# image-rs/deflate-rs

Measured on AMD Instinct MI355X. Metric: MB/s raw input encoded (Compression::Default) + compressed size vs ref, higher is better.
Workload: dtype u8; 1 GPU; enwik8 = enwik8-like synthetic text (tests/datagen.py text_like; --enwik8 PATH takes the real file): 100000000 bytes per GPU, Compression::Default, stream-exact (P1); bytes_per_gpu=100000000, level=Compression::Default, parallelism=shard1

## Files before the change

### __graft_entry__.py

```python
import os
import subprocess
import sys

ROOT = os.path.dirname(os.path.abspath(__file__))
PKG = os.path.join(ROOT, "deflate-rs_amd")
for p in (PKG, os.path.join(ROOT, "tests")):
    if p not in sys.path:
        sys.path.insert(0, p)


def _have_hipcc():
    return os.path.exists("/opt/rocm/bin/hipcc")


def build():
    env = dict(os.environ)
    lib = os.path.join(PKG, "libmi355deflate.so")
    if _have_hipcc():
        subprocess.check_call(["make", "-C", PKG, "-s"], env=env)
        subprocess.check_call(["make", "-C", PKG, "-s", "debug"], env=env)
    elif not os.path.exists(lib):
        raise RuntimeError("hipcc not found and no prebuilt libmi355deflate.so present")
    subprocess.check_call(["make", "-C", os.path.join(ROOT, "oracle"), "-s"], env=env)
    subprocess.check_call(["make", "-C", os.path.join(ROOT, "tests", "hostsim"), "-s"], env=env)
    subprocess.check_call(["make", "-C", os.path.join(ROOT, "tests", "inflcheck"), "-s"], env=env)
    subprocess.check_call(["make", "-C", os.path.join(ROOT, "tests", "inflwrite"), "-s"], env=env)
    subprocess.check_call(["make", "-C", os.path.join(ROOT, "tests", "infltable"), "-s"], env=env)
    subprocess.check_call(["make", "-C", os.path.join(ROOT, "tests", "inflindex"), "-s"], env=env)
    subprocess.check_call(["make", "-C", os.path.join(ROOT, "tests", "inflmembers"), "-s"], env=env)
    subprocess.check_call(["make", "-C", os.path.join(ROOT, "tests", "inflbig"), "-s"], env=env)
    subprocess.check_call(["make", "-C", os.path.join(ROOT, "tests", "inflseek"), "-s"], env=env)
    subprocess.check_call(["make", "-C", os.path.join(ROOT, "tests", "inflcut"), "-s"], env=env)
    import deflate_amd

    L = deflate_amd.load()
    for name in deflate_amd.EXPORTED:
        getattr(L, name)
    assert L.mi355_deflate_version() >= 100


def smoke():
    import zlib

    import deflate_amd
    import oracle_binding as ob

    pg = os.path.join(ROOT, "tests", "golden", "ref_inputs", "pg11.txt")
    data = open(pg, "rb").read()
    ctx = deflate_amd.Context(0)
    ctx.config(deflate_amd.Context.CFG_STAGE_CLOCKS, 1)
    out = ctx.encode(data, deflate_amd.Compression.Default)
    ref = ob.encode(data, level=ob.DEFAULT)
    assert out == ref, "HIP path differs from the oracle on pg11.txt (%d vs %d bytes)" % (len(out), len(ref))
    d = zlib.decompressobj(-15)
    assert d.decompress(out) + d.flush() == data
    z = ctx.encode(data[:70000], deflate_amd.Compression.Default, wrapper=1)
    assert zlib.decompress(z) == data[:70000]
    assert z == ob.encode(data[:70000], level=ob.DEFAULT, wrapper=1)
    info = ctx.info()
    print("smoke ok: pg11.txt %d -> %d bytes, %d blocks, match %.3f ms" %
          (len(data), len(out), info["n_blocks"], info["match_ms"]))


if __name__ == "__main__":
    build()
# ... 3 lines not shown
```

### deflate-rs_amd/csrc/deflate_batch.inc

```
namespace mi355 {

struct BatchItem {
    const uint8_t* in;
    uint32_t n, K0, nb_max;
    uint32_t q1_check;
    uint32_t out_words;
    uint32_t bit_base;
    uint32_t gz_off, gz_len;
    uint32_t *M, *Mq;
    uint16_t *adv, *S, *B;
    uint32_t *E0, *tokbuf, *cnt, *xs, *badmap, *fixlist, *base, *tend, *pb, *bstart, *q13, *dtok, *ll_freq, *d_freq, *seg_ends;
    BlockTab tab;
    BlockHeader* hdr;
    BlockPlan* plan;
    DevState* st;
    uint8_t* out;
};
enum : uint32_t { BS_SORT, BS_WALK, BS_RLE, BS_ADV, BS_EMIT, BS_COMPACT, BS_HIST, BS_HEADER, BS_PACK, BS_ADLER, BS_CRC, BS_N };
struct BatchArgs {
    const BatchItem* it;
    const uint32_t* pre;
    uint32_t n_items;
};
__device__ __forceinline__ uint32_t batch_locate(const BatchArgs& a, uint32_t stage, uint32_t& local, uint32_t& count) {
    const uint32_t* pre = a.pre + (size_t)stage * (a.n_items + 1);
    const uint32_t i = __builtin_amdgcn_readfirstlane(batch_item_of(pre, a.n_items, blockIdx.x));
    local = blockIdx.x - pre[i];
    count = pre[i + 1] - pre[i];
    return i;
}
__device__ __forceinline__ HashOverride batch_no_override() { return HashOverride{0, 0, 0, 0, 0, nullptr, 0, nullptr, 0, nullptr}; }

template <int MODE>
__global__ __launch_bounds__(1024) void kb_sort(BatchArgs bat_, uint32_t dbl) {
    uint32_t local, count;
    const BatchItem& it = bat_.it[batch_locate(bat_, BS_SORT, local, count)];
    k_sort_body<MODE>(local, it.in, it.n, batch_no_override(), it.S, it.B, 0u, dbl,
                      SortInit{reinterpret_cast<uint32_t*>(it.st), (uint32_t)(sizeof(DevScalars) / 4), it.seg_ends, it.n});
}

template <bool HAS_Q, bool SINGLE>
__global__ __launch_bounds__(M3T) __attribute__((amdgpu_waves_per_eu(4, 4))) void kb_walk(BatchArgs bat_, uint32_t checks, uint32_t checks_q,
                                                                                       uint32_t split) {
    __shared__ __attribute__((aligned(256))) uint4 s_T[M3_TABLE_U4];
    __shared__ uint32_t s_next;
    uint32_t local, count;
    const BatchItem& it = bat_.it[batch_locate(bat_, BS_WALK, local, count)];
    const uint32_t e = local / split, part = local % split;
    const SegEnds sg{it.seg_ends, 1u};
    const int aligned16 = (reinterpret_cast<uintptr_t>(it.in) & 15) == 0 ? 1 : 0;
    uint32_t* const ms = split == 1 ? walk_borrows(it.tokbuf, it.K0) : nullptr;
    uint32_t* const mqs = (HAS_Q && split == 1) ? it.dtok : nullptr;
    uint32_t* const Mq = HAS_Q ? it.Mq : nullptr;
    if (MI355_SWZ_BANKS && __builtin_amdgcn_readfirstlane((int)it.B[(size_t)e * BSTRIDE + WINDOW_SIZE + 2]))
        m3_epoch<HAS_Q, true, SINGLE>(s_T, s_next, e, part, it.in, it.n, it.S, it.B, it.M, Mq, checks, checks_q, aligned16, sg,
                                      batch_no_override(), split, ms, mqs, &it.st->sort_bad);
    else
        m3_epoch<HAS_Q, false, SINGLE>(s_T, s_next, e, part, it.in, it.n, it.S, it.B, it.M, Mq, checks, checks_q, aligned16, sg,
                                       batch_no_override(), split, ms, mqs, &it.st->sort_bad);
}

template <bool RLE>
__global__ __launch_bounds__(256) void kb_nohash(BatchArgs bat_) {
    uint32_t local, count;
    const BatchItem& it = bat_.it[batch_locate(bat_, BS_RLE, local, count)];
    if (local == 0) {
        uint32_t* const sc = reinterpret_cast<uint32_t*>(it.st);
        for (uint32_t i = threadIdx.x; i < (uint32_t)(sizeof(DevScalars) / 4); i += 256) sc[i] = 0;
        if (threadIdx.x == 0) *it.seg_ends = it.n;
    }
    if (RLE) {
        k_rle_body(local, it.in, it.n, it.M, it.adv, SegEnds{it.seg_ends, 1u});
    } else {
        const uint32_t lo = local * RT, hi = local + 1 == count ? ((it.n + 64 + 3) & ~3u) : lo + RT;
        for (uint32_t i = lo + threadIdx.x * 4; i < hi; i += 256 * 4) *reinterpret_cast<uint4*>(it.M + i) = make_uint4(0, 0, 0, 0);
    }
}

__global__ __launch_bounds__(256) void kb_adv(BatchArgs bat_, ParseCfg cfg) {
    uint32_t local, count;
    const BatchItem& it = bat_.it[batch_locate(bat_, BS_ADV, local, count)];
    k_adv_body(local, it.n, it.M, cfg.use_quarter ? it.Mq : nullptr, cfg, it.adv, SegEnds{it.seg_ends, 1u}, 0u);
}

template <bool STEPS>
__global__ __launch_bounds__(256) void kb_emit(BatchArgs bat_, ParseCfg cfg) {
    constexpr int MODE = 1;
    uint32_t local, count;
    const BatchItem& it = bat_.it[batch_locate(bat_, BS_EMIT, local, count)];
    const uint8_t* in = it.in;
    uint32_t n = it.n, K = it.K0;
    const uint32_t* M = it.M;
// ... 851 lines not shown
```

### deflate-rs_amd/csrc/deflate_host.inc

```
#include <dlfcn.h>
#include <hsa/hsa.h>
#include <hsa/hsa_ext_amd.h>
#include <stdio.h>
#include <stdlib.h>
#include <string.h>

#include <algorithm>
#include <chrono>
#include <mutex>
#include <string>
#include <vector>

#include "../../include/mi355_deflate.h"

using namespace mi355;

extern "C" size_t mi355_deflate_bound_ex(size_t n, int wrapper, size_t hdr_len, size_t n_flush);

namespace {

struct Level {
    uint32_t count;
    uint64_t usize;
    uint16_t* X;
// ... 527 lines not shown
    static const bool single_env = !(getenv("MI355_M3_SINGLE") && getenv("MI355_M3_SINGLE")[0] == '0');
    const uint32_t cus = n_cu ? n_cu : 256u;
    const uint32_t split = match3_split(n_ep, n_cu);
    return WalkPlan{split, single_env && split >= MI355_M3_SPLIT_MAX && n_ep * split * 2 <= cus};
}

void launch_walk(mi355_deflate_ctx* c, hipStream_t st, const uint8_t* d_in, uint32_t n32, const uint16_t* S, Workspace& w, const ParseCfg& cfg,
                 int aligned16, SegEnds sg, const HashOverride& ov, uint32_t e_first, uint32_t ne) {
    const WalkPlan plan = walk_plan(ne, c->n_cu);
    const uint32_t split = plan.split, cq = cfg_cq(cfg);
    const bool has_q = cfg_has_q(cfg);
    uint32_t* const borrowed = walk_borrows(w.tokbuf, w.K0);
    uint32_t* const ms = split == 1 ? borrowed : nullptr;
    uint32_t* const mqs = split == 1 ? w.dtok : nullptr;
    if (MI355_SWZ_BANKS && ne * split <= M3_BOTH_UNITS) {
        const bool single = plan.single;
        const uint32_t sp = single ? split * 2 : split;
        uint32_t* const ms1 = sp == 1 ? borrowed : nullptr;
        uint32_t* const mqs1 = sp == 1 ? w.dtok : nullptr;
#define MI355_BOTH(Q, SNG, mq, mqs, cqv)                                                                                       \
    hipLaunchKernelGGL((k_match3_both<Q, SNG>), dim3(ne * sp), dim3(M3T), 0, st, d_in, n32, S, w.buckets, w.M, mq, cfg.checks, cqv, \
                       aligned16, sg, ov, e_first, sp, ms1, mqs, sort_bad_flag(c))
        if (has_q && single)
            MI355_BOTH(true, true, w.Mq, mqs1, cq);
        else if (has_q)
            MI355_BOTH(true, false, w.Mq, mqs1, cq);
        else if (single)
            MI355_BOTH(false, true, (uint32_t*)nullptr, (uint32_t*)nullptr, 0u);
        else
            MI355_BOTH(false, false, (uint32_t*)nullptr, (uint32_t*)nullptr, 0u);
#undef MI355_BOTH
        return;
    }
    if (has_q)
        hipLaunchKernelGGL(k_match3<true>, dim3(ne * split), dim3(M3T), 0, st, d_in, n32, S, w.buckets, w.M, w.Mq, cfg.checks, cq,
                           aligned16, sg, ov, e_first, split, ms, mqs, sort_bad_flag(c));
    else
        hipLaunchKernelGGL(k_match3<false>, dim3(ne * split), dim3(M3T), 0, st, d_in, n32, S, w.buckets, w.M, (uint32_t*)nullptr,
                           cfg.checks, 0u, aligned16, sg, ov, e_first, split, ms, (uint32_t*)nullptr, sort_bad_flag(c));
    if (MI355_SWZ_BANKS) {
        const uint32_t units = ne * split, cus = c->n_cu ? c->n_cu : 256u;
        const uint32_t grid = (MI355_SWZ_PERSISTENT && units > cus) ? cus : units;
        if (has_q)
            hipLaunchKernelGGL(k_match3_swz<true>, dim3(grid), dim3(M3T), 0, st, d_in, n32, S, w.buckets, w.M, w.Mq, cfg.checks, cq,
                               aligned16, sg, ov, e_first, units, split, ms, mqs, sort_bad_flag(c));
        else
            hipLaunchKernelGGL(k_match3_swz<false>, dim3(grid), dim3(M3T), 0, st, d_in, n32, S, w.buckets, w.M, (uint32_t*)nullptr,
                               cfg.checks, 0u, aligned16, sg, ov, e_first, units, split, ms, (uint32_t*)nullptr, sort_bad_flag(c));
    }
}

struct SegRange {
    uint32_t seg_hi;
    Piece piece;
    const uint8_t* d_in;
    uint32_t n, pos0, n_total;
    uint32_t runup0;
    SegEnds sg;
    const uint16_t* steps;
    uint32_t* E0;
    uint32_t* xs;
    uint32_t* fixlist;
    uint32_t* n_fix;
    uint32_t* scan_part;
    uint32_t* tend;
    uint32_t* pb;
};

void launch_spec_emit(hipStream_t st, const Workspace& w, const ParseCfg& cfg, const SegRange& r) {
    const SpecFix fx{r.fixlist, w.badmap, r.n_fix};
    MI355_LAUNCH_EMIT(1, r.steps, dim3(cdiv(r.seg_hi - r.piece.seg_lo, 4)), st, r.d_in, r.n, r.seg_hi, w.M, cfg.use_quarter ? w.Mq : nullptr, cfg,
                       r.steps, r.E0, w.tokbuf, w.cnt, r.pos0, r.n_total, r.sg, r.xs, fx, r.runup0, r.piece.seg_lo);
// ... 1606 lines not shown
```

### deflate-rs_amd/csrc/deflate_kernels.hip

```cpp
#include <hip/hip_runtime.h>
#include <stdint.h>

#include <type_traits>

#ifdef MI355_MATCH_STATS
__device__ unsigned long long g_mstats[16];
__device__ unsigned long long g_sstats[16];
#define MI355_STAT_DECL uint32_t stat_[8] = {0, 0, 0, 0, 0, 0, 0, 0};
#define MI355_STAT(i, v) stat_[i] += (v);
#define MI355_STAT_FLUSH(policy)                                                          \
    for (int i_ = 0; i_ < 8; i_++) atomicAdd(&g_mstats[i_], (unsigned long long)stat_[i_]); \
    atomicMax((policy).wgmax, stat_[0]);                                                  \
    if ((threadIdx.x & 63) == 0) {                                                        \
        unsigned long long t_ = wall_clock64();                                           \
        atomicMax((policy).wgend, t_);                                                    \
        atomicAdd((policy).wgsum, t_ - (policy).t0);                                      \
    }
#endif
#include "stages.h"

namespace mi355 {

struct GBytes {
    const uint8_t* d;
// ... 807 lines not shown
                very += nb <= MI355_SWZ_BANKS / 2 ? 1u : 0u;
            }
            bool banks_few = few >= 2 || very >= 1;
#ifdef MI355_DEBUG_HOOKS
            if (force_swz) banks_few = force_swz == 1u;
#endif
            Bg[(size_t)e * BSTRIDE + WINDOW_SIZE + 2] = (J >= 1024 && banks_few && dbl) ? 1 : 0;
        }
    }
    uint4* out = reinterpret_cast<uint4*>(Sg + (size_t)e * WINDOW_SIZE);
    const uint4* fin = reinterpret_cast<const uint4*>(sH);
    for (uint32_t k = tid; k < (J + 7) / 8; k += 1024) {
        const uint4 v = fin[k];
        out[k] = make_uint4(v.x << dbl, v.y << dbl, v.z << dbl, v.w << dbl);
    }
}
template <int MODE>
__global__ __launch_bounds__(1024) void k_sort(const uint8_t* __restrict__ in, uint32_t n, HashOverride ov,
                                               uint16_t* __restrict__ Sg, uint16_t* __restrict__ Bg, uint32_t e0, uint32_t dbl,
                                               SortInit init) {
    k_sort_body<MODE>(blockIdx.x, in, n, ov, Sg, Bg, e0, dbl, init);
}

#ifdef MI355_MATCH_STATS
#define M2_CNT(i, v) \
    if (((MI355_MATCH_STATS) & 2) || (i) == 0 || (i) == 4) m2c[i] += (uint32_t)(v);
#define M2_T0 uint32_t m2t = ((MI355_MATCH_STATS) & 1) ? (uint32_t)__builtin_readcyclecounter() : 0u;
#define M2_T(i)                                                      \
    if ((MI355_MATCH_STATS) & 1) {                                   \
        const uint32_t t_ = (uint32_t)__builtin_readcyclecounter();  \
        m2c[i] += t_ - m2t;                                          \
        m2t = t_;                                                    \
    }
#else
#define M2_CNT(i, v)
#define M2_T0
#define M2_T(i)
#endif

constexpr uint32_t M3T = 1024;
constexpr uint32_t M3_PAIRS = 2 * WINDOW_SIZE + 258 + 14;

template <bool SWZ>
struct PairWinT {
    const uint16_t* sb;
    uint32_t tbase;
    typedef __attribute__((address_space(3))) const uint16_t* lds_u16;
    enum : uint32_t { SH = 1 };
    __device__ uint32_t key_at(uint32_t a) const { return *(lds_u16)(SWZ ? m3_swz(a) : a); }
    __device__ void load16(uint32_t pos, uint32_t* q) const {
        typedef uint32_t u32x2 __attribute__((ext_vector_type(2)));
        u32x2 d0, d1, d2, d3, d4;
        const uint32_t a8 = (tbase + 2 * pos) & ~7u;
        if (SWZ) {
            asm volatile(
                "ds_read_b64 %0, %5\n\t"
                "ds_read_b64 %1, %6\n\t"
                "ds_read_b64 %2, %7\n\t"
                "ds_read_b64 %3, %8\n\t"
                "ds_read_b64 %4, %9\n\t"
                "s_waitcnt lgkmcnt(0)"
                : "=&v"(d0), "=&v"(d1), "=&v"(d2), "=&v"(d3), "=&v"(d4)
                : "v"(m3_swz(a8)), "v"(m3_swz(a8 + 8)), "v"(m3_swz(a8 + 16)), "v"(m3_swz(a8 + 24)), "v"(m3_swz(a8 + 32))
                : "memory");
        } else
        asm volatile(
            "ds_read_b64 %0, %5\n\t"
            "ds_read_b64 %1, %5 offset:8\n\t"
            "ds_read_b64 %2, %5 offset:16\n\t"
            "ds_read_b64 %3, %5 offset:24\n\t"
// ... 151 lines not shown
        "s_mov_b64 %[cx], exec\n\t" \
        "s_mov_b64 exec, %[cy]\n\t" \
        MF_TEST8("y", "7", "6", "5", "4", "3", "2", "1", "0") \
        "s_mov_b64 %[cy], exec\n\t" \
        "s_branch .Lmf_end%=\n\t" \
        ".Lmf_xonly%=:\n\t" \
        MF_ONE(RD8, "x", "wx", "cx", "v[56:59]", "v[60:63]", "v56", "v57", "v58", "v59", "v60", "v61", "v62", "v63") \
        "s_branch .Lmf_end%=\n\t" \
        ".Lmf_yonly%=:\n\t" \
        MF_ONE(RD8, "y", "wy", "cy", "v[64:67]", "v[68:71]", "v64", "v65", "v66", "v67", "v68", "v69", "v70", "v71") \
        ".Lmf_end%=:\n\t" \
        "s_waitcnt vmcnt(0)\n\t" \
        "s_mov_b64 exec, %[save]\n\t" \
        : MF_OPS(x, x), MF_OPS(y, y), [save] "=&s"(save), [cx] "=&s"(cx), [cy] "=&s"(cy) \
        : MF_INS(x, x), MF_INS(y, y), [sb] "s"(sb8), [wx] "s"(walkx), [wy] "s"(walky) \
        : "vcc", "scc", "memory", "v56", "v57", "v58", "v59", "v60", "v61", "v62", "v63", "v64", "v65", "v66", "v67", "v68", "v69", \
          "v70", "v71"); \
    *stillx = cx; \
    *stilly = cy; \
}
MS_STEPS_DUAL_DEF(ms_steps_dual, MF_RD8_0)
MS_STEPS_DUAL_DEF(ms_steps_dual_swz, MF_RD8_1)
#undef MF_ONE

constexpr uint32_t ADV_TILE = 1024, ADV_HALO = 260;
struct TileM {
    const uint32_t* t;
    __device__ uint32_t operator()(uint32_t r) const { return t[r]; }
};
__device__ __forceinline__ uint32_t rel_end(const SegEnds& sg, uint64_t base, uint32_t r) {
    const uint64_t e = (uint64_t)seg_end(sg, base + r) - base;
    return e > 0xFFFFFFFFull ? 0xFFFFFFFFu : (uint32_t)e;
}
template <bool HAS_Q, bool SWZ, bool SINGLE = false>
__device__ __forceinline__ void m3_epoch(uint4* s_T, uint32_t& s_next, const uint32_t e, const uint32_t part, const uint8_t* __restrict__ in, uint32_t n,
                                         const uint16_t* __restrict__ Sg, const uint16_t* __restrict__ Bg, uint32_t* __restrict__ M,
                                         uint32_t* __restrict__ Mq, uint32_t checks, uint32_t checks_q, int in_aligned16, SegEnds sg,
                                         HashOverride ov, uint32_t split, uint32_t* __restrict__ Ms, uint32_t* __restrict__ Mqs,
                                         uint32_t* __restrict__ sort_bad) {
    constexpr uint32_t pair = SINGLE ? 1u : 2u;
    const uint32_t tid = threadIdx.x, lane = tid & 63;
#ifdef MI355_MATCH_STATS
    uint32_t m2c[16] = {0, 0, 0, 0, 0, 0, 0, 0, 0, 0, 0, 0, 0, 0, 0, 0};
#endif
    M2_T0
    const uint64_t E = (uint64_t)e * WINDOW_SIZE;
    const uint64_t wbase = e ? E - WINDOW_SIZE : 0;
    const uint32_t wbytes = (uint32_t)(E - wbase) + WINDOW_SIZE + 258 + 14;
    const uint32_t tb0 = (uint32_t)(uintptr_t)(__attribute__((address_space(3))) uint4*)s_T;
    for (uint32_t w = tid; w < wbytes / 16; w += M3T) {
        const uint64_t g = wbase + 16ull * w;
        uint32_t t[5] = {0, 0, 0, 0, 0};
        if (in_aligned16 && g + 20 <= n) {
            const uint4 v = *reinterpret_cast<const uint4*>(in + g);
            t[0] = v.x;
            t[1] = v.y;
            t[2] = v.z;
            t[3] = v.w;
            t[4] = *reinterpret_cast<const uint32_t*>(in + g + 16);
        } else {
            for (int b = 0; b < 17; b++)
                if (g + b < n) t[b >> 2] |= (uint32_t)in[g + b] << (8 * (b & 3));
        }
        uint32_t o[8];
#pragma unroll
        for (int k = 0; k < 4; k++) {
            o[2 * k] = __builtin_amdgcn_perm(t[k], t[k], 0x02010100u);
            o[2 * k + 1] = __builtin_amdgcn_perm(t[k + 1], t[k], 0x04030302u);
        }
        if (SWZ) {
            typedef __attribute__((address_space(3))) uint64_t* lds_u64;
            const uint32_t a = tb0 + 32u * w;
#pragma unroll
            for (int k = 0; k < 4; k++) *(lds_u64)m3_swz(a + 8u * k) = (uint64_t)o[2 * k] | ((uint64_t)o[2 * k + 1] << 32);
        } else {
            s_T[2 * w] = make_uint4(o[0], o[1], o[2], o[3]);
            s_T[2 * w + 1] = make_uint4(o[4], o[5], o[6], o[7]);
        }
    }
    const uint32_t J = epoch_active(n, E);
    const uint32_t nbat = (J + 63) / 64;
    const uint32_t b_lo = (uint32_t)((uint64_t)nbat * part / split), b_hi = (uint32_t)((uint64_t)nbat * (part + 1) / split);
    if (tid == 0) s_next = b_lo;
    if (part == 0 && tid < 2) {
        const uint64_t p = E + J + tid;
        if (p < n && p < E + WINDOW_SIZE) {
            M[p] = 0;
            if (HAS_Q) Mq[p] = 0;
        }
    }
    __syncthreads();
    const uint32_t tbase = tb0;
    const uint32_t bias = (uint32_t)(E - wbase);
    const uint16_t* sbase = Sg + (size_t)e * WINDOW_SIZE - WINDOW_SIZE;
    const uint16_t* own = Sg + (size_t)e * WINDOW_SIZE;
    const uint16_t* Bown = Bg + (size_t)e * BSTRIDE;
    const uint16_t* Bprev = Bown - BSTRIDE;
    TileLimit lim{sg, wbase, sg.m == 1 ? (uint32_t)(sg.ends[0] - wbase) : 0u};
    M2_T(10)
    uint32_t unordered = 0;
    auto set_up = [&](const auto& win, SwG<HAS_Q>& st, uint32_t b, bool have, uint32_t* srel_out, uint32_t before0, uint32_t* last_out,
                      uint32_t skip, uint32_t budget, uint32_t budget_q) -> bool {
        const uint32_t j = b * 64 + lane;
        const bool valid = have && j < J;
        uint32_t raw = 0, srel = 0, ob = 0, pb0 = 0, pb1 = 0, prel = bias, nrel = bias;
        if (valid) {
            raw = (uint32_t)own[j];
            srel = raw >> 1;
            prel = bias + srel;
            const uint32_t v = win.load32(prel);
            const uint32_t ab = rewarm_ab(ov, E + srel, v & 0xff, (v >> 8) & 0xff);
            const uint32_t h = hash3(ab & 0xff, ab >> 8, (v >> 16) & 0xff);
            ob = Bown[h];
            if (e) {
                pb0 = Bprev[h];
// ... 29 lines not shown
            M2_CNT(2, 1)
            M2_CNT(3, __popcll(dropped))
            swg_service<decltype(run1)::value>(st, win, tbase, checks_q, dropped, any & dropped, asel, st.offb + back);
        }
    };
    uint32_t* const Mo = Ms ? Ms : M;
    uint32_t* const Mqo = Ms ? Mqs : Mq;
    const uint16_t* sb8u;
    {
        const uint64_t v = (uint64_t)(uintptr_t)(sbase - 4);
        const uint32_t lo = (uint32_t)__builtin_amdgcn_readfirstlane((int)(uint32_t)v);
        const uint32_t hi = (uint32_t)__builtin_amdgcn_readfirstlane((int)(uint32_t)(v >> 32));
        sb8u = (const uint16_t*)(uintptr_t)(((uint64_t)hi << 32) | lo);
    }
    auto walk_all = [&](auto run1) {
        constexpr bool RUN1 = decltype(run1)::value;
        const PairWinT<SWZ> win{sbase, tbase};
        uint32_t pxat = ~0u, pxm = 0, pxq = 0, pyat = ~0u, pym = 0, pyq = 0;
        for (;;) {
            uint32_t b = 0;
            if (lane == 0) b = atomicAdd(&s_next, pair);
            b = (uint32_t)__builtin_amdgcn_readfirstlane((int)b);
            if (b >= b_hi) break;
            SwG<HAS_Q> sx, sy;
            uint32_t srx, sry;
            uint32_t lastx, lasty;
            const uint32_t front = b ? (uint32_t)own[(uint32_t)__builtin_amdgcn_readfirstlane((int)(b * 64 - 1))] : 0u;
            const uint32_t half = (pair == 1u && checks >= 16u) ? checks / 2u : 0u;
            const bool vx = set_up(win, sx, b, true, &srx, front, &lastx, 0u, half ? half : checks, checks_q);
            const bool vy = half ? set_up(win, sy, b, true, &sry, front, &lasty, half, checks - half, 0u)
                                 : set_up(win, sy, b + 1, pair == 2u && b + 1 < b_hi, &sry, lastx, &lasty, 0u, checks, checks_q);
            (void)lasty;
            M2_CNT(0, 2)
            M2_T(8)
            if (pxat != ~0u) {
                Mo[E + pxat] = pxm;
                if (HAS_Q) Mqo[E + pxat] = pxq;
            }
            if (pyat != ~0u) {
                Mo[E + pyat] = pym;
                if (HAS_Q) Mqo[E + pyat] = pyq;
            }
            {
                const uint64_t dx = swg_first(sx, win, 8u), dy = swg_first(sy, win, 8u);
                if (dx) swg_service<RUN1>(sx, win, tbase, checks_q, dx, dx, sx.a0, sx.offb + 16u);
                if (dy) swg_service<RUN1>(sy, win, tbase, checks_q, dy, dy, sy.a0, sy.offb + 16u);
                M2_CNT(2, 2)
                M2_CNT(3, __popcll(dx) + __popcll(dy))
                M2_T(9)
            }
            for (;;) {
                const uint64_t wx = sx.walk, wy = sy.walk;
                if ((wx | wy) == 0) break;
                M2_CNT(1, 1)
                M2_CNT(7, __popcll(wx) + __popcll(wy))
                uint64_t cx, cy;
                if (SWZ)
                    ms_steps_dual_swz(sx, sy, sb8u, wx, wy, &cx, &cy);
                else
                    ms_steps_dual(sx, sy, sb8u, wx, wy, &cx, &cy);
                M2_T(12)
                sx.walk = cx;
                sy.walk = cy;
                uint64_t dx, dy;
                asm("s_andn2_b64 %0, %2, %3\n\ts_andn2_b64 %1, %4, %5" : "=&s"(dx), "=&s"(dy) : "s"(wx), "s"(cx), "s"(wy), "s"(cy) : "scc");
                if (dx) settle(run1, win, sx, dx);
                if (dy) settle(run1, win, sy, dy);
                M2_T(9)
            }
            swg_result(sx, &pxm, &pxq);
            swg_result(sy, &pym, &pyq);
            pxat = vx ? (Ms ? b * 64 + lane : srx) : ~0u;
            pyat = vy ? (Ms ? b * 64 + 64 + lane : sry) : ~0u;
            if (half) {
                pxm = m_len(pym) > m_len(pxm) ? pym : pxm;
                pyat = ~0u;
            }
            M2_T(13)
        }
        if (pxat != ~0u) {
            Mo[E + pxat] = pxm;
            if (HAS_Q) Mqo[E + pxat] = pxq;
        }
        if (pyat != ~0u) {
            Mo[E + pyat] = pym;
            if (HAS_Q) Mqo[E + pyat] = pyq;
        }
    };
    if (!SWZ && __builtin_amdgcn_readfirstlane((int)Bown[WINDOW_SIZE + 1]))
        walk_all(std::true_type{});
    else
        walk_all(std::false_type{});
    if (__builtin_amdgcn_ballot_w64(unordered != 0) != 0 && lane == 0) atomicOr(sort_bad, 1u);
    M2_T(11)
    if (Ms) {
        uint32_t* const lm = reinterpret_cast<uint32_t*>(s_T);
        const uint32_t cnt = (uint32_t)((uint64_t)n - E < (uint64_t)WINDOW_SIZE ? (uint64_t)n - E : (uint64_t)WINDOW_SIZE);
        for (int pass = 0; pass < (HAS_Q ? 2 : 1); pass++) {
            const uint32_t* src = pass ? Mqs : Ms;
            uint32_t* dst = pass ? Mq : M;
            __syncthreads();
            for (uint32_t j = tid; j < J; j += M3T) lm[(uint32_t)own[j] >> 1] = src[E + j];
            if (tid < 2 && J + tid < cnt) lm[J + tid] = 0;
            __syncthreads();
            for (uint32_t i = tid * 4; i < cnt; i += M3T * 4) {
                if (i + 4 <= cnt) {
                    *reinterpret_cast<uint4*>(dst + E + i) = *reinterpret_cast<const uint4*>(lm + i);
                } else {
                    for (uint32_t k = i; k < cnt; k++) dst[E + k] = lm[k];
                }
            }
        }
    }
    M2_T(14)
    M2_CNT(4, 1)
#ifdef MI355_MATCH_STATS
    if (lane == 0)
        for (int i = 0; i < 16; i++) atomicAdd(&g_mstats[i], (unsigned long long)m2c[i]);
#endif
}

constexpr uint32_t M3_TABLE_U4 = (M3_PAIRS * 2 + 255) / 256 * 16;
template <bool HAS_Q>
__global__ __launch_bounds__(M3T) __attribute__((amdgpu_waves_per_eu(4, 4))) void k_match3(const uint8_t* __restrict__ in, uint32_t n, const uint16_t* __restrict__ Sg,
                                                const uint16_t* __restrict__ Bg, uint32_t* __restrict__ M,
                                                uint32_t* __restrict__ Mq, uint32_t checks, uint32_t checks_q, int in_aligned16,
                                                SegEnds sg, HashOverride ov, uint32_t e0, uint32_t split, uint32_t* __restrict__ Ms,
                                                uint32_t* __restrict__ Mqs, uint32_t* __restrict__ sort_bad) {
    __shared__ __attribute__((aligned(256))) uint4 s_T[M3_TABLE_U4];
    __shared__ uint32_t s_next;
    const uint32_t e = e0 + blockIdx.x / split, part = blockIdx.x % split;
    if (MI355_SWZ_BANKS && __builtin_amdgcn_readfirstlane((int)Bg[(size_t)e * BSTRIDE + WINDOW_SIZE + 2])) return;
    m3_epoch<HAS_Q, false>(s_T, s_next, e, part, in, n, Sg, Bg, M, Mq, checks, checks_q, in_aligned16, sg, ov, split, Ms, Mqs, sort_bad);
}
template <bool HAS_Q>
__global__ __launch_bounds__(M3T) __attribute__((amdgpu_waves_per_eu(4, 4))) void k_match3_swz(const uint8_t* __restrict__ in, uint32_t n, const uint16_t* __restrict__ Sg,
                                                const uint16_t* __restrict__ Bg, uint32_t* __restrict__ M,
                                                uint32_t* __restrict__ Mq, uint32_t checks, uint32_t checks_q, int in_aligned16,
                                                SegEnds sg, HashOverride ov, uint32_t e0, uint32_t units, uint32_t split,
                                                uint32_t* __restrict__ Ms, uint32_t* __restrict__ Mqs, uint32_t* __restrict__ sort_bad) {
    __shared__ __attribute__((aligned(256))) uint4 s_T[M3_TABLE_U4];
    __shared__ uint32_t s_next;
#if MI355_SWZ_PERSISTENT
    for (uint32_t u = blockIdx.x; u < units; u += gridDim.x) {
        const uint32_t e = e0 + u / split;
        if (!__builtin_amdgcn_readfirstlane((int)Bg[(size_t)e * BSTRIDE + WINDOW_SIZE + 2])) continue;
        __syncthreads();
        m3_epoch<HAS_Q, true>(s_T, s_next, e, u % split, in, n, Sg, Bg, M, Mq, checks, checks_q, in_aligned16, sg, ov, split, Ms, Mqs, sort_bad);
    }
#else
    (void)units;
    const uint32_t e = e0 + blockIdx.x / split;
    if (!__builtin_amdgcn_readfirstlane((int)Bg[(size_t)e * BSTRIDE + WINDOW_SIZE + 2])) return;
    m3_epoch<HAS_Q, true>(s_T, s_next, e, blockIdx.x % split, in, n, Sg, Bg, M, Mq, checks, checks_q, in_aligned16, sg, ov, split, Ms, Mqs, sort_bad);
#endif
}

#ifndef MI355_M3_BOTH_UNITS
#define MI355_M3_BOTH_UNITS 256
#endif
constexpr uint32_t M3_BOTH_UNITS = MI355_M3_BOTH_UNITS;
template <bool HAS_Q, bool SINGLE>
__global__ __launch_bounds__(M3T) __attribute__((amdgpu_waves_per_eu(4, 4))) void k_match3_both(const uint8_t* __restrict__ in, uint32_t n, const uint16_t* __restrict__ Sg,
                                                const uint16_t* __restrict__ Bg, uint32_t* __restrict__ M,
                                                uint32_t* __restrict__ Mq, uint32_t checks, uint32_t checks_q, int in_aligned16,
                                                SegEnds sg, HashOverride ov, uint32_t e0, uint32_t split, uint32_t* __restrict__ Ms,
                                                uint32_t* __restrict__ Mqs, uint32_t* __restrict__ sort_bad) {
    __shared__ __attribute__((aligned(256))) uint4 s_T[M3_TABLE_U4];
    __shared__ uint32_t s_next;
    const uint32_t e = e0 + blockIdx.x / split, part = blockIdx.x % split;
    if (MI355_SWZ_BANKS && __builtin_amdgcn_readfirstlane((int)Bg[(size_t)e * BSTRIDE + WINDOW_SIZE + 2]))
        m3_epoch<HAS_Q, true, SINGLE>(s_T, s_next, e, part, in, n, Sg, Bg, M, Mq, checks, checks_q, in_aligned16, sg, ov, split, Ms, Mqs, sort_bad);
    else
        m3_epoch<HAS_Q, false, SINGLE>(s_T, s_next, e, part, in, n, Sg, Bg, M, Mq, checks, checks_q, in_aligned16, sg, ov, split, Ms, Mqs, sort_bad);
}

constexpr uint32_t RT = 4096;
constexpr uint32_t RLE_UNITS = RT / 16 + 17;
constexpr uint32_t RLE_BYTES = 16 + RLE_UNITS * 16;
__device__ __forceinline__ void k_rle_body(uint32_t bx_, const uint8_t* __restrict__ in, uint32_t n, uint32_t* __restrict__ R,
                                           uint16_t* __restrict__ adv, SegEnds sg) {
    __shared__ __attribute__((aligned(16))) uint8_t s[RLE_BYTES];
    __shared__ uint32_t eb[RLE_UNITS + 1];
    __shared__ __attribute__((aligned(16))) uint32_t so[RT];
    __shared__ __attribute__((aligned(16))) uint16_t sa[RT];
    const uint32_t tid = threadIdx.x;
    const uint64_t E = (uint64_t)bx_ * RT;
    const bool al = (reinterpret_cast<uintptr_t>(in) & 15) == 0;
    for (uint32_t k = tid; k < RLE_BYTES / 16; k += 256) {
        const int64_t g0 = (int64_t)E - 16 + 16 * (int64_t)k;
        uint4 v = make_uint4(0, 0, 0, 0);
        if (al && g0 >= 0 && (uint64_t)g0 + 16 <= n) {
            v = *reinterpret_cast<const uint4*>(in + g0);
        } else {
            uint32_t t[4] = {0, 0, 0, 0};
            for (int b = 0; b < 16; b++) {
                const int64_t g = g0 + b;
                if (g >= 0 && (uint64_t)g < n) t[b >> 2] |= (uint32_t)in[g] << (8 * (b & 3));
            }
            v = make_uint4(t[0], t[1], t[2], t[3]);
        }
        *reinterpret_cast<uint4*>(s + 16 * k) = v;
    }
    __syncthreads();
    auto unit_bits = [&](uint32_t u) -> uint32_t {
        const uint32_t* w = reinterpret_cast<const uint32_t*>(s + 16 * u + 12);
        const uint32_t d0 = w[0], d1 = w[1], d2 = w[2], d3 = w[3], d4 = w[4];
// ... 1669 lines not shown
```

### deflate-rs_amd/csrc/stages.h

```cpp
#ifndef MI355_DEFLATE_STAGES_H
#define MI355_DEFLATE_STAGES_H

#include <stdint.h>

#if defined(__HIPCC__)
#define MI355_HD __host__ __device__ __forceinline__
#else
#define MI355_HD inline
#endif

namespace mi355 {

enum : uint32_t {
    WINDOW_SIZE = 32768,
    MIN_MATCH = 3,
    MAX_MATCH = 258,
    TOO_FAR = 8192,
    MAX_BUFFER_LENGTH = 31744,
    MAX_STORED_BLOCK_LENGTH = 32767,
    NUM_LL = 286,
    NUM_DIST = 30,
    END_OF_BLOCK = 256,
    MAX_JUMP = 520,
    ZONE = 576,
// ... 586 lines not shown
        s.hq = s.hq | cap;
    }
    const lane_flag imp = hit & lf_of(len > s.bm1 + 1);
    const uint32_t delta = lf_me(imp) ? len - 1 - s.bm1 : 0u;
    s.bestd = lf_me(imp) ? s.prel - cpos : s.bestd;
    s.bm1 += delta;
    s.bb2 += delta << W::SH;
    s.lowa2 += delta << W::SH;
    const lane_flag full = imp & lf_of(len == s.maxlen);
    const uint32_t pr = w.key_at(tbase + ((s.prel + s.bm1) << W::SH));
    s.probe = lf_me(imp) ? pr : s.probe;
    s.offb = lf_me(hit) ? ho - 2 : s.offb;
    const lane_flag more = lf_of((int32_t)s.offb >= (int32_t)s.endb);
    const lane_flag resume = lf_and_not(hit & more, full);
    const lane_flag sw = lf_and_not(lf_and_not(dropped, resume), full) & s.has2;
    if (lf_any(sw)) {
        if (HAS_Q) s.hoq = lf_me(sw) ? s.hoq2 : s.hoq;
        s.offb = lf_me(sw) ? s.offb2 : s.offb;
        s.endb = lf_me(sw) ? s.endb2 : s.endb;
        s.bb2 = lf_me(sw) ? tbase + (s.bm1 << W::SH) : s.bb2;
        s.has2 = lf_and_not(s.has2, sw);
    }
    s.walk = s.walk | resume | sw;
}

template <bool HAS_Q>
MI355_HD void swg_result(const SwG<HAS_Q>& s, uint32_t* m, uint32_t* mq) {
    const uint32_t r = m_pack(s.bestd ? s.bm1 + 1 : 0, s.bestd);
    *m = r;
    *mq = (HAS_Q && lf_me(s.hq)) ? s.mq : r;
}

MI355_HD uint32_t m3_swz(uint32_t a) { return a ^ ((a >> 5) & 0xF8u); }

template <class Bytes>
MI355_HD uint32_t rle_run(const Bytes& by, uint64_t p, uint64_t n) {
    if (p == 0) return 0;
    uint32_t prev = by(p - 1);
    uint64_t cap = n - p < (uint64_t)MAX_MATCH ? n - p : (uint64_t)MAX_MATCH;
    uint32_t c = 0;
    while (c < cap && by(p + c) == prev) c++;
    return c;
}

struct SegEnds {
    const uint32_t* ends;
    uint32_t m;
};
MI355_HD uint32_t seg_end(const SegEnds& sg, uint64_t p) {
    if (sg.m == 1) return sg.ends[0];
    uint32_t lo = 0, hi = sg.m - 1;
    while (lo < hi) {
        uint32_t mid = (lo + hi) >> 1;
        if (sg.ends[mid] > p)
            hi = mid;
        else
            lo = mid + 1;
    }
    return sg.ends[lo];
}

struct ParseCfg {
    uint32_t mode;
    uint32_t checks;
    uint32_t lazy_lt;
    uint32_t use_quarter;
// ... 571 lines not shown
```

Baseline: 23540 MB/s.

## Prefetch match-window staging loads early and warm caches for the next epoch

The match3 kernels now issue the first window-staging load (and the run/mark flags as one combined load) before branching, stage later rounds ahead in registers, and touch the sort keys for the first batch early. After the walk, each block also issues loads that warm L2 for the epoch a stride ahead (input bytes, sort keys, bucket flags). The aim is to hide global-memory latency at the start of each epoch. The cost is extra register pressure and redundant loads, including for blocks that exit early.

```diff
diff --git a/__graft_entry__.py b/__graft_entry__.py
--- a/__graft_entry__.py
+++ b/__graft_entry__.py
@@ -31,6 +31,7 @@
     subprocess.check_call(["make", "-C", os.path.join(ROOT, "tests", "inflbig"), "-s"], env=env)
     subprocess.check_call(["make", "-C", os.path.join(ROOT, "tests", "inflseek"), "-s"], env=env)
     subprocess.check_call(["make", "-C", os.path.join(ROOT, "tests", "inflcut"), "-s"], env=env)
+    subprocess.check_call(["make", "-C", os.path.join(ROOT, "tests", "matchwarm"), "-s"], env=env)
     import deflate_amd
 
     L = deflate_amd.load()
diff --git a/deflate-rs_amd/csrc/deflate_batch.inc b/deflate-rs_amd/csrc/deflate_batch.inc
--- a/deflate-rs_amd/csrc/deflate_batch.inc
+++ b/deflate-rs_amd/csrc/deflate_batch.inc
@@ -52,12 +52,15 @@
     uint32_t* const ms = split == 1 ? walk_borrows(it.tokbuf, it.K0) : nullptr;
     uint32_t* const mqs = (HAS_Q && split == 1) ? it.dtok : nullptr;
     uint32_t* const Mq = HAS_Q ? it.Mq : nullptr;
-    if (MI355_SWZ_BANKS && __builtin_amdgcn_readfirstlane((int)it.B[(size_t)e * BSTRIDE + WINDOW_SIZE + 2]))
+    const M3Flags fl = m3_flags(it.B, e);
+    const M3Head hd = m3_head(it.in, it.n, aligned16, it.B, e, threadIdx.x);
+    const uint32_t run = fl.run;
+    if (MI355_SWZ_BANKS && __builtin_amdgcn_readfirstlane((int)fl.mark))
         m3_epoch<HAS_Q, true, SINGLE>(s_T, s_next, e, part, it.in, it.n, it.S, it.B, it.M, Mq, checks, checks_q, aligned16, sg,
-                                      batch_no_override(), split, ms, mqs, &it.st->sort_bad);
+                                      batch_no_override(), split, ms, mqs, &it.st->sort_bad, hd, run);
     else
         m3_epoch<HAS_Q, false, SINGLE>(s_T, s_next, e, part, it.in, it.n, it.S, it.B, it.M, Mq, checks, checks_q, aligned16, sg,
-                                       batch_no_override(), split, ms, mqs, &it.st->sort_bad);
+                                       batch_no_override(), split, ms, mqs, &it.st->sort_bad, hd, run);
 }
 
 template <bool RLE>
diff --git a/deflate-rs_amd/csrc/deflate_host.inc b/deflate-rs_amd/csrc/deflate_host.inc
--- a/deflate-rs_amd/csrc/deflate_host.inc
+++ b/deflate-rs_amd/csrc/deflate_host.inc
@@ -583,12 +583,13 @@
 #undef MI355_BOTH
         return;
     }
+    const uint32_t warm_stride = c->n_cu ? c->n_cu : 256u, e_end = e_first + ne;
     if (has_q)
         hipLaunchKernelGGL(k_match3<true>, dim3(ne * split), dim3(M3T), 0, st, d_in, n32, S, w.buckets, w.M, w.Mq, cfg.checks, cq,
-                           aligned16, sg, ov, e_first, split, ms, mqs, sort_bad_flag(c));
+                           aligned16, sg, ov, e_first, split, ms, mqs, sort_bad_flag(c), warm_stride, e_end);
     else
         hipLaunchKernelGGL(k_match3<false>, dim3(ne * split), dim3(M3T), 0, st, d_in, n32, S, w.buckets, w.M, (uint32_t*)nullptr,
-                           cfg.checks, 0u, aligned16, sg, ov, e_first, split, ms, (uint32_t*)nullptr, sort_bad_flag(c));
+                           cfg.checks, 0u, aligned16, sg, ov, e_first, split, ms, (uint32_t*)nullptr, sort_bad_flag(c), warm_stride, e_end);
     if (MI355_SWZ_BANKS) {
         const uint32_t units = ne * split, cus = c->n_cu ? c->n_cu : 256u;
         const uint32_t grid = (MI355_SWZ_PERSISTENT && units > cus) ? cus : units;
diff --git a/deflate-rs_amd/csrc/deflate_kernels.hip b/deflate-rs_amd/csrc/deflate_kernels.hip
--- a/deflate-rs_amd/csrc/deflate_kernels.hip
+++ b/deflate-rs_amd/csrc/deflate_kernels.hip
@@ -863,10 +863,17 @@
         m2c[i] += t_ - m2t;                                          \
         m2t = t_;                                                    \
     }
+#define M2_T_SETUP     \
+    if (pxat == ~0u && pyat == ~0u) { \
+        M2_T(15)       \
+    } else {           \
+        M2_T(8)        \
+    }
 #else
 #define M2_CNT(i, v)
 #define M2_T0
 #define M2_T(i)
+#define M2_T_SETUP
 #endif
 
 constexpr uint32_t M3T = 1024;
@@ -1084,12 +1091,126 @@
     const uint64_t e = (uint64_t)seg_end(sg, base + r) - base;
     return e > 0xFFFFFFFFull ? 0xFFFFFFFFu : (uint32_t)e;
 }
+#ifndef MI355_M3_EARLY_FLAGS
+#define MI355_M3_EARLY_FLAGS 1
+#endif
+#ifndef MI355_M3_STAGE_AHEAD
+#define MI355_M3_STAGE_AHEAD 1
+#endif
+#ifndef MI355_M3_WARM_FIRST
+#define MI355_M3_WARM_FIRST 1
+#endif
+#ifndef MI355_M3_WARM_NEXT
+#define MI355_M3_WARM_NEXT 2
+#endif
+struct M3Flags {
+    uint32_t run, mark;
+};
+__device__ __forceinline__ M3Flags m3_flags(const uint16_t* __restrict__ Bg, uint32_t e) {
+    uint32_t both;
+    __builtin_memcpy(&both, Bg + (size_t)e * BSTRIDE + WINDOW_SIZE + 1, 4);
+    return M3Flags{both & 0xffffu, both >> 16};
+}
+__device__ __forceinline__ uint64_t m3_wbase(uint32_t e) { return e ? (uint64_t)e * WINDOW_SIZE - WINDOW_SIZE : 0; }
+__device__ __forceinline__ bool m3_whole_item(uint32_t n, int in_aligned16, uint64_t g) { return in_aligned16 && g + 20 <= n; }
+__device__ __forceinline__ void m3_fetch(const uint8_t* __restrict__ in, uint32_t n, int in_aligned16, uint64_t g, uint32_t (&t)[5]) {
+    t[0] = t[1] = t[2] = t[3] = t[4] = 0;
+    if (m3_whole_item(n, in_aligned16, g)) {
+        const uint4 v = *reinterpret_cast<const uint4*>(in + g);
+        t[0] = v.x;
+        t[1] = v.y;
+        t[2] = v.z;
+        t[3] = v.w;
+        t[4] = *reinterpret_cast<const uint32_t*>(in + g + 16);
+    } else {
+        for (int b = 0; b < 17; b++)
+            if (g + b < n) t[b >> 2] |= (uint32_t)in[g + b] << (8 * (b & 3));
+    }
+}
+struct M3Head {
+    uint4 v;
+    uint32_t t4;
+    bool whole;
+};
+__device__ __forceinline__ M3Head m3_head(const uint8_t* __restrict__ in, uint32_t n, int in_aligned16, const uint16_t* __restrict__ Bg,
+                                          uint32_t e, uint32_t w, bool inside = true) {
+    M3Head h;
+    const uint64_t g = m3_wbase(e) + 16ull * w;
+    h.whole = inside && m3_whole_item(n, in_aligned16, g);
+    const uint8_t* src = h.whole ? in + g : reinterpret_cast<const uint8_t*>(Bg + (size_t)e * BSTRIDE + WINDOW_SIZE);
+    h.v = *reinterpret_cast<const uint4*>(src);
+    h.t4 = *reinterpret_cast<const uint32_t*>(src + 16);
+    return h;
+}
+constexpr uint32_t M3_ROUNDS = (M3_PAIRS / 16 + M3T - 1) / M3T;
+template <bool SWZ, uint32_t PAIR>
+__device__ __forceinline__ void m3_stage(uint32_t tb0, const uint8_t* __restrict__ in, uint32_t n, int in_aligned16,
+                                         const uint16_t* __restrict__ Sg, const uint16_t* __restrict__ Bg, uint32_t e, const M3Head& hd,
+                                         uint32_t J, uint32_t b_lo) {
+    const uint32_t tid = threadIdx.x, lane = tid & 63;
+    const uint64_t wbase = m3_wbase(e);
+    const uint32_t wbytes = (uint32_t)((uint64_t)e * WINDOW_SIZE - wbase) + WINDOW_SIZE + 258 + 14;
+    M3Head it[M3_ROUNDS];
+    it[0] = hd;
+#if MI355_M3_STAGE_AHEAD
+#pragma unroll
+    for (uint32_t r = 1; r < M3_ROUNDS; r++) it[r] = m3_head(in, n, in_aligned16, Bg, e, tid + r * M3T, tid + r * M3T < wbytes / 16);
+#endif
+#if MI355_M3_WARM_FIRST
+    const uint16_t* const se = Sg + (size_t)e * WINDOW_SIZE;
+    const uint32_t j0 = (b_lo + PAIR * (tid >> 6)) * 64 + lane;
+    const uint32_t warm_a = se[j0 < J ? j0 : 0u], warm_b = se[(PAIR == 2 && j0 + 64 < J) ? j0 + 64 : 0u];
+    const uint32_t warm_c = se[(j0 && j0 < J) ? j0 - 1 : 0u];
+#endif
+    auto put = [&](uint32_t w, const uint32_t (&t)[5]) {
+        uint32_t o[8];
+#pragma unroll
+        for (int k = 0; k < 4; k++) {
+            o[2 * k] = __builtin_amdgcn_perm(t[k], t[k], 0x02010100u);
+            o[2 * k + 1] = __builtin_amdgcn_perm(t[k + 1], t[k], 0x04030302u);
+        }
+        if (SWZ) {
+            typedef __attribute__((address_space(3))) uint64_t* lds_u64;
+            const uint32_t a = tb0 + 32u * w;
+#pragma unroll
+            for (int k = 0; k < 4; k++) *(lds_u64)m3_swz(a + 8u * k) = (uint64_t)o[2 * k] | ((uint64_t)o[2 * k + 1] << 32);
+        } else {
+            typedef uint32_t u32x4 __attribute__((ext_vector_type(4)));
+            typedef __attribute__((address_space(3))) u32x4* lds_u4;
+            *(lds_u4)(tb0 + 32u * w) = u32x4{o[0], o[1], o[2], o[3]};
+            *(lds_u4)(tb0 + 32u * w + 16u) = u32x4{o[4], o[5], o[6], o[7]};
+        }
+    };
+#pragma unroll
+    for (uint32_t r = 0; r < M3_ROUNDS; r++) {
+#if !MI355_M3_STAGE_AHEAD
+        if (r) it[r].whole = false;
+#endif
+        if (it[r].whole) {
+            const uint32_t t[5] = {it[r].v.x, it[r].v.y, it[r].v.z, it[r].v.w, it[r].t4};
+            put(tid + r * M3T, t);
+        }
+    }
+#pragma unroll
+    for (uint32_t r = 0; r < M3_ROUNDS; r++) {
+        const uint32_t w = tid + r * M3T;
+        if (w < wbytes / 16 && !it[r].whole) {
+            uint32_t t[5];
+            m3_fetch(in, n, in_aligned16, wbase + 16ull * w, t);
+            put(w, t);
+        }
+    }
+#if MI355_M3_WARM_FIRST
+    asm volatile("" ::"v"(warm_a), "v"(warm_b), "v"(warm_c));
+#endif
+}
 template <bool HAS_Q, bool SWZ, bool SINGLE = false>
 __device__ __forceinline__ void m3_epoch(uint4* s_T, uint32_t& s_next, const uint32_t e, const uint32_t part, const uint8_t* __restrict__ in, uint32_t n,
                                          const uint16_t* __restrict__ Sg, const uint16_t* __restrict__ Bg, uint32_t* __restrict__ M,
                                          uint32_t* __restrict__ Mq, uint32_t checks, uint32_t checks_q, int in_aligned16, SegEnds sg,
                                          HashOverride ov, uint32_t split, uint32_t* __restrict__ Ms, uint32_t* __restrict__ Mqs,
-                                         uint32_t* __restrict__ sort_bad) {
+                                         uint32_t* __restrict__ sort_bad, const M3Head& hd, uint32_t run_flag,
+                                         uint32_t warm_stride = 0, uint32_t e_end = 0) {
     constexpr uint32_t pair = SINGLE ? 1u : 2u;
     const uint32_t tid = threadIdx.x, lane = tid & 63;
 #ifdef MI355_MATCH_STATS
@@ -1097,42 +1218,13 @@
 #endif
     M2_T0
     const uint64_t E = (uint64_t)e * WINDOW_SIZE;
-    const uint64_t wbase = e ? E - WINDOW_SIZE : 0;
+    const uint64_t wbase = m3_wbase(e);
     const uint32_t wbytes = (uint32_t)(E - wbase) + WINDOW_SIZE + 258 + 14;
     const uint32_t tb0 = (uint32_t)(uintptr_t)(__attribute__((address_space(3))) uint4*)s_T;
-    for (uint32_t w = tid; w < wbytes / 16; w += M3T) {
-        const uint64_t g = wbase + 16ull * w;
-        uint32_t t[5] = {0, 0, 0, 0, 0};
-        if (in_aligned16 && g + 20 <= n) {
-            const uint4 v = *reinterpret_cast<const uint4*>(in + g);
-            t[0] = v.x;
-            t[1] = v.y;
-            t[2] = v.z;
-            t[3] = v.w;
-            t[4] = *reinterpret_cast<const uint32_t*>(in + g + 16);
-        } else {
-            for (int b = 0; b < 17; b++)
-                if (g + b < n) t[b >> 2] |= (uint32_t)in[g + b] << (8 * (b & 3));
-        }
-        uint32_t o[8];
-#pragma unroll
-        for (int k = 0; k < 4; k++) {
-            o[2 * k] = __builtin_amdgcn_perm(t[k], t[k], 0x02010100u);
-            o[2 * k + 1] = __builtin_amdgcn_perm(t[k + 1], t[k], 0x04030302u);
-        }
-        if (SWZ) {
-            typedef __attribute__((address_space(3))) uint64_t* lds_u64;
-            const uint32_t a = tb0 + 32u * w;
-#pragma unroll
-            for (int k = 0; k < 4; k++) *(lds_u64)m3_swz(a + 8u * k) = (uint64_t)o[2 * k] | ((uint64_t)o[2 * k + 1] << 32);
-        } else {
-            s_T[2 * w] = make_uint4(o[0], o[1], o[2], o[3]);
-            s_T[2 * w + 1] = make_uint4(o[4], o[5], o[6], o[7]);
-        }
-    }
     const uint32_t J = epoch_active(n, E);
     const uint32_t nbat = (J + 63) / 64;
     const uint32_t b_lo = (uint32_t)((uint64_t)nbat * part / split), b_hi = (uint32_t)((uint64_t)nbat * (part + 1) / split);
+    m3_stage<SWZ, pair>(tb0, in, n, in_aligned16, Sg, Bg, e, hd, J, b_lo);
     if (tid == 0) s_next = b_lo;
     if (part == 0 && tid < 2) {
         const uint64_t p = E + J + tid;
@@ -1228,7 +1320,7 @@
                                  : set_up(win, sy, b + 1, pair == 2u && b + 1 < b_hi, &sry, lastx, &lasty, 0u, checks, checks_q);
             (void)lasty;
             M2_CNT(0, 2)
-            M2_T(8)
+            M2_T_SETUP
             if (pxat != ~0u) {
                 Mo[E + pxat] = pxm;
                 if (HAS_Q) Mqo[E + pxat] = pxq;
@@ -1283,11 +1375,29 @@
             if (HAS_Q) Mqo[E + pyat] = pyq;
         }
     };
-    if (!SWZ && __builtin_amdgcn_readfirstlane((int)Bown[WINDOW_SIZE + 1]))
+    if (!SWZ && __builtin_amdgcn_readfirstlane((int)run_flag))
         walk_all(std::true_type{});
     else
         walk_all(std::false_type{});
     if (__builtin_amdgcn_ballot_w64(unordered != 0) != 0 && lane == 0) atomicOr(sort_bad, 1u);
+#if MI355_M3_WARM_NEXT
+    uint32_t warm_next = 0;
+    if (warm_stride) {
+        const M3Warm wr = m3_warm_ranges(e, e_end, n, warm_stride, split, BSTRIDE, MI355_M3_WARM_NEXT == 2);
+        if (wr.on) {
+            constexpr uint32_t LINE = 128, s_lines = M3_WARM_S * 2 / LINE;
+            const uint32_t in_lines = (uint32_t)((wr.in_hi - wr.in_lo + LINE - 1) / LINE);
+            if (tid < in_lines) {
+                warm_next = in[wr.in_lo + (uint64_t)LINE * tid];
+            } else if (tid < in_lines + 2 * s_lines) {
+                const uint32_t k = tid - in_lines;
+                warm_next = (Sg + (k < s_lines ? wr.s_lo[0] : wr.s_lo[1]))[(k % s_lines) * (LINE / 2)];
+            } else if (tid == in_lines + 2 * s_lines) {
+                warm_next = Bg[wr.b_lo];
+            }
+        }
+    }
+#endif
     M2_T(11)
     if (Ms) {
         uint32_t* const lm = reinterpret_cast<uint32_t*>(s_T);
@@ -1308,6 +1418,9 @@
             }
         }
     }
+#if MI355_M3_WARM_NEXT
+    asm volatile("" ::"v"(warm_next));
+#endif
     M2_T(14)
     M2_CNT(4, 1)
 #ifdef MI355_MATCH_STATS
@@ -1322,12 +1435,20 @@
                                                 const uint16_t* __restrict__ Bg, uint32_t* __restrict__ M,
                                                 uint32_t* __restrict__ Mq, uint32_t checks, uint32_t checks_q, int in_aligned16,
                                                 SegEnds sg, HashOverride ov, uint32_t e0, uint32_t split, uint32_t* __restrict__ Ms,
-                                                uint32_t* __restrict__ Mqs, uint32_t* __restrict__ sort_bad) {
+                                                uint32_t* __restrict__ Mqs, uint32_t* __restrict__ sort_bad, uint32_t warm_stride,
+                                                uint32_t e_end) {
     __shared__ __attribute__((aligned(256))) uint4 s_T[M3_TABLE_U4];
     __shared__ uint32_t s_next;
     const uint32_t e = e0 + blockIdx.x / split, part = blockIdx.x % split;
-    if (MI355_SWZ_BANKS && __builtin_amdgcn_readfirstlane((int)Bg[(size_t)e * BSTRIDE + WINDOW_SIZE + 2])) return;
-    m3_epoch<HAS_Q, false>(s_T, s_next, e, part, in, n, Sg, Bg, M, Mq, checks, checks_q, in_aligned16, sg, ov, split, Ms, Mqs, sort_bad);
+    const M3Flags fl = m3_flags(Bg, e);
+    if (!MI355_M3_EARLY_FLAGS && MI355_SWZ_BANKS && __builtin_amdgcn_readfirstlane((int)fl.mark)) return;
+    const M3Head hd = m3_head(in, n, in_aligned16, Bg, e, threadIdx.x);
+    if (MI355_M3_EARLY_FLAGS && MI355_SWZ_BANKS && __builtin_amdgcn_readfirstlane((int)fl.mark)) {
+        asm volatile("" ::"v"(hd.v.x), "v"(hd.t4));
+        return;
+    }
+    m3_epoch<HAS_Q, false>(s_T, s_next, e, part, in, n, Sg, Bg, M, Mq, checks, checks_q, in_aligned16, sg, ov, split, Ms, Mqs, sort_bad, hd,
+                           fl.run, warm_stride, e_end);
 }
 template <bool HAS_Q>
 __global__ __launch_bounds__(M3T) __attribute__((amdgpu_waves_per_eu(4, 4))) void k_match3_swz(const uint8_t* __restrict__ in, uint32_t n, const uint16_t* __restrict__ Sg,
@@ -1340,15 +1461,17 @@
 #if MI355_SWZ_PERSISTENT
     for (uint32_t u = blockIdx.x; u < units; u += gridDim.x) {
         const uint32_t e = e0 + u / split;
-        if (!__builtin_amdgcn_readfirstlane((int)Bg[(size_t)e * BSTRIDE + WINDOW_SIZE + 2])) continue;
+        if (!__builtin_amdgcn_readfirstlane((int)m3_flags(Bg, e).mark)) continue;
+        const M3Head hd = m3_head(in, n, in_aligned16, Bg, e, threadIdx.x);
         __syncthreads();
-        m3_epoch<HAS_Q, true>(s_T, s_next, e, u % split, in, n, Sg, Bg, M, Mq, checks, checks_q, in_aligned16, sg, ov, split, Ms, Mqs, sort_bad);
+        m3_epoch<HAS_Q, true>(s_T, s_next, e, u % split, in, n, Sg, Bg, M, Mq, checks, checks_q, in_aligned16, sg, ov, split, Ms, Mqs, sort_bad, hd, 0u);
     }
 #else
     (void)units;
     const uint32_t e = e0 + blockIdx.x / split;
-    if (!__builtin_amdgcn_readfirstlane((int)Bg[(size_t)e * BSTRIDE + WINDOW_SIZE + 2])) return;
-    m3_epoch<HAS_Q, true>(s_T, s_next, e, blockIdx.x % split, in, n, Sg, Bg, M, Mq, checks, checks_q, in_aligned16, sg, ov, split, Ms, Mqs, sort_bad);
+    if (!__builtin_amdgcn_readfirstlane((int)m3_flags(Bg, e).mark)) return;
+    const M3Head hd = m3_head(in, n, in_aligned16, Bg, e, threadIdx.x);
+    m3_epoch<HAS_Q, true>(s_T, s_next, e, blockIdx.x % split, in, n, Sg, Bg, M, Mq, checks, checks_q, in_aligned16, sg, ov, split, Ms, Mqs, sort_bad, hd, 0u);
 #endif
 }
 
@@ -1365,10 +1488,13 @@
     __shared__ __attribute__((aligned(256))) uint4 s_T[M3_TABLE_U4];
     __shared__ uint32_t s_next;
     const uint32_t e = e0 + blockIdx.x / split, part = blockIdx.x % split;
-    if (MI355_SWZ_BANKS && __builtin_amdgcn_readfirstlane((int)Bg[(size_t)e * BSTRIDE + WINDOW_SIZE + 2]))
-        m3_epoch<HAS_Q, true, SINGLE>(s_T, s_next, e, part, in, n, Sg, Bg, M, Mq, checks, checks_q, in_aligned16, sg, ov, split, Ms, Mqs, sort_bad);
+    const M3Flags fl = m3_flags(Bg, e);
+    const M3Head hd = m3_head(in, n, in_aligned16, Bg, e, threadIdx.x);
+    const uint32_t run = fl.run;
+    if (MI355_SWZ_BANKS && __builtin_amdgcn_readfirstlane((int)fl.mark))
+        m3_epoch<HAS_Q, true, SINGLE>(s_T, s_next, e, part, in, n, Sg, Bg, M, Mq, checks, checks_q, in_aligned16, sg, ov, split, Ms, Mqs, sort_bad, hd, run);
     else
-        m3_epoch<HAS_Q, false, SINGLE>(s_T, s_next, e, part, in, n, Sg, Bg, M, Mq, checks, checks_q, in_aligned16, sg, ov, split, Ms, Mqs, sort_bad);
+        m3_epoch<HAS_Q, false, SINGLE>(s_T, s_next, e, part, in, n, Sg, Bg, M, Mq, checks, checks_q, in_aligned16, sg, ov, split, Ms, Mqs, sort_bad, hd, run);
 }
 
 constexpr uint32_t RT = 4096;
diff --git a/deflate-rs_amd/csrc/stages.h b/deflate-rs_amd/csrc/stages.h
--- a/deflate-rs_amd/csrc/stages.h
+++ b/deflate-rs_amd/csrc/stages.h
@@ -642,6 +642,31 @@
 }
 
 MI355_HD uint32_t m3_swz(uint32_t a) { return a ^ ((a >> 5) & 0xF8u); }
+
+constexpr uint32_t M3_WARM_S = 2048;
+constexpr uint32_t M3_WARM_B = 8;
+struct M3Warm {
+    uint32_t on, e;
+    uint64_t in_lo, in_hi;
+    int64_t s_lo[2];
+    uint64_t b_lo;
+};
+MI355_HD M3Warm m3_warm_ranges(uint32_t e, uint32_t n_ep, uint64_t n, uint32_t stride, uint32_t split, uint32_t bstride,
+                               bool with_prev) {
+    M3Warm r = {0u, 0u, 0ull, 0ull, {0, 0}, 0ull};
+    const uint64_t et = (uint64_t)e + (split ? stride / split : 0u);
+    if (stride == 0 || split == 0 || stride / split == 0 || et >= n_ep || et * WINDOW_SIZE >= n) return r;
+    const uint64_t E = et * WINDOW_SIZE;
+    r.on = 1;
+    r.e = (uint32_t)et;
+    r.in_lo = (with_prev && et) ? E - WINDOW_SIZE : E;
+    r.in_hi = E + WINDOW_SIZE + 258 + 14;
+    if (r.in_hi > n) r.in_hi = n;
+    r.s_lo[0] = (int64_t)E;
+    r.s_lo[1] = (int64_t)E - WINDOW_SIZE;
+    r.b_lo = et * bstride + WINDOW_SIZE;
+    return r;
+}
 
 template <class Bytes>
 MI355_HD uint32_t rle_run(const Bytes& by, uint64_t p, uint64_t n) {
```

After: 23690 MB/s, median of 6. Within noise of the previous version (+0.6%).
